# ZAX130/SmileCode

Measured on AMD Instinct MI355X. Metric: volume-pairs/sec (160x192x160) fwd+bwd, higher is better.
Workload: dtype f32; 1 GPU; ModeT 160x192x160 fp32, batch=1/GPU, full train step NCC+Grad3d fwd+bwd+Adam-amsgrad; global_batch=1, parallelism=dp1, allreduce=one flat all-reduce after backward

## Files before the change

### smilecode_amd/_lib.py

```python
from __future__ import annotations

import ctypes as C
import os
import re

_HERE = os.path.dirname(os.path.abspath(__file__))
LIB_PATH = os.environ.get("MODET_HIP_LIB") or os.path.join(_HERE, "lib", "libmodet_hip.so")
HEADER_PATH = os.path.join(os.path.dirname(_HERE), "include", "modet_hip.h")

P, I, I64, F, SZ = C.c_void_p, C.c_int, C.c_int64, C.c_float, C.c_size_t

class LeafJob(C.Structure):
    _fields_ = [("part", P), ("outer", I64), ("outer_stride", I64), ("rows", I64), ("row_stride", I64),
                ("col_group_stride", I64), ("ncols", I), ("col_group", I), ("dst", P * 4), ("n", I * 4)]


SIGNATURES = {
    "modet_hip_version": (I, []),
    "modet_hip_strerror": (C.c_char_p, [I]),
    "modet_qk_fwd": (I, [P, P, P, P, I, I, I, I, I, I, P]),
    "modet_qk_bwd_ws_bytes": (SZ, [I, I, I, I, I]),
    "modet_qk_bwd": (I, [P, P, P, P, P, P, P, SZ, I, I, I, I, I, I, P]),
    "modet_qk_fwd_f64": (I, [P, P, P, P, I, I, I, I, I, I, P]),
    "modet_qk_bwd_ws_bytes_f64": (SZ, [I, I, I, I, I]),
# ... 114 lines not shown
def _header(name):
    return os.path.join(os.path.dirname(_HERE), "include", name)


FAMILIES = {
    "core": (HEADER_PATH, SIGNATURES),
    "mind": (_header("modet_hip_losses.h"), {
        "modet_mind_ws_bytes": (SZ, [I, I, I, I, I]),
        "modet_mind_descriptor": (I, [P, P, P, SZ, I, I, I, I, I, I, P]),
        "modet_mind_fwd_bwd": (I, [P, P, P, P, P, SZ, I, I, I, I, I, I, F, P]),
    }),
    "mi": (_header("modet_hip_mi.h"), {
        "modet_mi_ws_bytes": (SZ, [I, I, I, I, I]),
        "modet_mi_fwd_bwd": (I, [P, P, P, P, P, P, SZ, I, I, I, I, I, F, F, F, F, P]),
        "modet_lmi_fwd_bwd": (I, [P, P, P, P, P, P, SZ, I, I, I, I, I, F, F, F, I, F, P]),
    }),
    "ssim": (_header("modet_hip_ssim.h"), {
        "modet_ssim_ws_bytes": (SZ, [I, I, I, I, I]),
        "modet_ssim_fwd_bwd": (I, [P, P, P, P, P, P, SZ, I, I, I, I, I, F, P]),
    }),
    "reg": (_header("modet_hip_reg.h"), {
        "modet_reg_ws_bytes": (SZ, [I, I, I, I, I, I]),
        "modet_reg_fwd_bwd": (I, [P, P, P, P, SZ, I, I, I, I, I, I, I, F, P]),
    }),
    "vecint": (_header("modet_hip_vecint.h"), {
        "modet_vecint_fwd": (I, [P, P, P, P, I, I, I, I, I, P]),
        "modet_vecint_ws_bytes": (SZ, [I, I, I, I, I, F]),
        "modet_vecint_bwd": (I, [P, P, P, P, P, P, SZ, I, I, I, I, I, F, P]),
    }),
    "surface": (_header("modet_hip_surface.h"), {
        "modet_surface_ws_bytes": (SZ, [I, I, I, I]),
        "modet_surface_distances": (I, [P, P, P, P, P, SZ, I, I, I, I, F, P]),
    }),
}
((LOSS_HEADER_PATH, LOSS_SIGNATURES), (MI_HEADER_PATH, MI_SIGNATURES), (SSIM_HEADER_PATH, SSIM_SIGNATURES),
 (REG_HEADER_PATH, REG_SIGNATURES), (VECINT_HEADER_PATH, VECINT_SIGNATURES)) = (FAMILIES[k] for k in ("mind", "mi", "ssim", "reg", "vecint"))

_lib = None


def header_symbols(path=None):
    txt = open(path or HEADER_PATH).read()
    txt = re.sub(r"/\*.*?\*/", "", txt, flags=re.S)
    return sorted(set(re.findall(r"\b(modet_[a-z0-9_]+)\s*\(", txt)))


def load():
    global _lib
    if _lib is not None:
        return _lib
    if not os.path.exists(LIB_PATH):
        raise RuntimeError(
            f"{LIB_PATH} not found: build it with `python -m smilecode_amd.build` "
            "(the ModeT hot path has no CPU / eager fallback)")
    lib = C.CDLL(LIB_PATH)
    for _, table in FAMILIES.values():
        for name, (res, args) in table.items():
            if not hasattr(lib, name) and os.environ.get("MODET_HIP_LIB"):
                continue
            fn = getattr(lib, name)
            fn.restype = res
            fn.argtypes = args
    _lib = lib
    return lib


# ... 8 lines not shown
```

### smilecode_amd/csrc/na.hip

```cpp
#include "common.h"
#include "drpb_reduce.h"
#include <cstdlib>

namespace {

constexpr int HD = 6;
constexpr int TZ = 4, TY = 4, TX = 16;
constexpr int HZ = TZ + 2, HY = TY + 2, HX = TX + 2;
constexpr int HVOX = HZ * HY * HX;
constexpr int NTHREADS = TZ * TY * TX;

struct TileGeom {
  int tiles_x, tiles_y, tiles_z;
};

__device__ __forceinline__ void tile_origin(int tile, const TileGeom g, int& z0, int& y0, int& x0) {
  const int tx = tile % g.tiles_x;
  const int t2 = tile / g.tiles_x;
  x0 = tx * TX;
  y0 = (t2 % g.tiles_y) * TY;
  z0 = (t2 / g.tiles_y) * TZ;
}

constexpr int KT_IT = (HVOX * 3 + NTHREADS - 1) / NTHREADS;
__device__ __forceinline__ float2 bf2_unpack(unsigned u) { return make_float2(__uint_as_float(u << 16), __uint_as_float(u & 0xffff0000u)); }
template <bool QK16 = false>
__device__ __forceinline__ void stage_k_load(float2 (&r)[KT_IT], const float* __restrict__ k, int64_t bbase, int z0, int y0,
                                             int x0, int D, int H, int W, int C, int hoff) {
  bool inside[KT_IT];
#pragma unroll
  for (int j = 0; j < KT_IT; ++j) {
    const int idx = min((int)threadIdx.x + j * NTHREADS, HVOX * 3 - 1);
    const int v = idx / 3, part = idx - v * 3;
    const int hx = v % HX, t = v / HX;
// ... 45 lines not shown
}

__device__ __forceinline__ void logits27(const float* __restrict__ kt, int lt, const float (&qs)[HD],
                                         const float* __restrict__ rpb_h, float (&lg)[27]) {
#pragma unroll
  for (int ki = 0; ki < 3; ++ki)
#pragma unroll
    for (int kj = 0; kj < 3; ++kj)
#pragma unroll
      for (int kk = 0; kk < 3; ++kk) {
        const int t = ki * 9 + kj * 3 + kk;
        float kv[HD];
        load6(kt + (lt + (ki * HY + kj) * HX + kk) * HD, kv);
        float s = rpb_h[t];
#pragma unroll
        for (int c = 0; c < HD; ++c) s = fmaf(qs[c], kv[c], s);
        lg[t] = s;
      }
}

__device__ __forceinline__ float softmax27(float (&lg)[27], float& m) {
  m = lg[0];
#pragma unroll
  for (int t = 1; t < 27; ++t) m = fmaxf(m, lg[t]);
  float s = 0.f;
#pragma unroll
  for (int t = 0; t < 27; ++t) {
    lg[t] = __expf(lg[t] - m);
    s += lg[t];
  }
  return 1.f / s;
}

template <bool QK16>
__global__ __launch_bounds__(NTHREADS) void na_fwd_kernel(const float* __restrict__ q, const float* __restrict__ k,
                                                          const float* __restrict__ rpb, float* __restrict__ out,
                                                          float* __restrict__ lse, int D, int H, int W, int heads,
                                                          float scale, TileGeom g) {
  __shared__ __attribute__((aligned(16))) float kt[HVOX * HD];
  __shared__ float rp[27];
  const int h = blockIdx.y, b = blockIdx.z;
  const int C = heads * HD;
  const int64_t V = (int64_t)D * H * W;
  int z0, y0, x0;
  tile_origin(blockIdx.x, g, z0, y0, x0);
  if (threadIdx.x < 27) rp[threadIdx.x] = rpb[h * 27 + threadIdx.x];
  stage_k_tile<QK16>(kt, k, (int64_t)b * V, z0, y0, x0, D, H, W, C, h * HD);
  __syncthreads();

  const int tx = threadIdx.x % TX, ty = (threadIdx.x / TX) % TY, tz = threadIdx.x / (TX * TY);
  const int z = z0 + tz, y = y0 + ty, x = x0 + tx;
  if (z >= D || y >= H || x >= W) return;
  const int64_t n = (int64_t)b * V + ((int64_t)z * H + y) * W + x;
  float qs[HD];
  load6g<QK16>(q, n * C + h * HD, qs);
#pragma unroll
  for (int c = 0; c < HD; ++c) qs[c] *= scale;
  float p[27];
  logits27(kt, (tz * HY + ty) * HX + tx, qs, rp, p);
  float mx;
  const float inv = softmax27(p, mx);
  if (lse) lse[n * heads + h] = mx - __logf(inv);
  float o0 = 0.f, o1 = 0.f, o2 = 0.f;
#pragma unroll
  for (int ki = 0; ki < 3; ++ki)
#pragma unroll
    for (int kj = 0; kj < 3; ++kj)
#pragma unroll
      for (int kk = 0; kk < 3; ++kk) {
        const float pv = p[ki * 9 + kj * 3 + kk];
        o0 += pv * (float)(ki - 1);
        o1 += pv * (float)(kj - 1);
        o2 += pv * (float)(kk - 1);
      }
  float* o = out + n * (heads * 3) + h * 3;
  o[0] = o0 * inv; o[1] = o1 * inv; o[2] = o2 * inv;
}

template <int N>
__device__ __forceinline__ void rs_step(float (&v)[32], int lane) {
  const bool up = (lane & N) != 0;
#pragma unroll
  for (int i = 0; i < N / 2; ++i) {
    const float keep = up ? v[i + N / 2] : v[i];
    const float send = up ? v[i] : v[i + N / 2];
    v[i] = keep + __shfl_xor(send, N, 64);
  }
}
__device__ __forceinline__ float wave_reduce_scatter32(const float (&v27)[27], int lane) {
  float v[32];
#pragma unroll
  for (int i = 0; i < 32; ++i) v[i] = i < 27 ? v27[i] : 0.f;
  rs_step<32>(v, lane); rs_step<16>(v, lane); rs_step<8>(v, lane); rs_step<4>(v, lane); rs_step<2>(v, lane);
  return v[0] + __shfl_xor(v[0], 1, 64);
}

constexpr int AUX = 5;

template <bool QK16>
__global__ __launch_bounds__(NTHREADS) void na_bwd_kernel(const float* __restrict__ q, const float* __restrict__ k,
                                                          const float* __restrict__ rpb, const float* __restrict__ out,
                                                          const float* __restrict__ lse, const float* __restrict__ dout,
                                                          float* __restrict__ dq, float* __restrict__ dk,
                                                          float* __restrict__ drpb_part, int D, int H, int W, int heads,
                                                          float scale, TileGeom g) {
  __shared__ __attribute__((aligned(16))) float kt[HVOX * HD];
  __shared__ __attribute__((aligned(16))) float qt[HVOX * HD];
  __shared__ float ax[HVOX * AUX];
  __shared__ float red[27 * (NTHREADS / 64)];
// ... 336 lines not shown
  const int lane = threadIdx.x & 63, wv = threadIdx.x >> 6;
  {
    const float r = wave_reduce_scatter32(dlv, lane);
    if ((lane & 1) == 0 && (lane >> 1) < 27) red[wv * 27 + (lane >> 1)] = r;
  }
  __syncthreads();
  if (threadIdx.x < 27) {
    float s = 0.f;
    for (int w = 0; w < NTHREADS / 64; ++w) s += red[w * 27 + threadIdx.x];
    const int64_t blk = ((int64_t)b * gridDim.y + h) * gridDim.x + blockIdx.x;
    a.drpb_part[blk * 27 + threadIdx.x] = s;
  }
}

struct NaMarchPlan { int tiles_x, tiles_y, nchunk, zc; bool on; };
inline NaMarchPlan na_march_plan(int B, int D, int H, int W, int heads, int hd) {
  NaMarchPlan p;
  p.tiles_x = cdiv(W, MX); p.tiles_y = cdiv(H, MY);
  p.on = hd == HD && (int64_t)D * H * W >= 1500000 && (int64_t)H * W * heads * HD * 4 < 0x7fffffffLL;
  const int cols = B * heads * p.tiles_x * p.tiles_y;
  int want = 2000;
#ifdef MODET_TUNING
  if (const char* e = getenv("MODET_NA_WGS")) want = atoi(e);
  if (const char* e = getenv("MODET_NA_MARCH")) p.on = p.on && e[0] != '0';
#endif
  int best = (want + cols - 1) / cols;
  const int maxn = D / 8 > 0 ? D / 8 : 1;
  best = best < 1 ? 1 : (best > maxn ? maxn : best);
  p.zc = cdiv(D, best);
  p.nchunk = cdiv(D, p.zc);
  return p;
}

constexpr int GC = 8;

__device__ __forceinline__ void stage_chunk(float* __restrict__ dst, const float* __restrict__ srcp, int64_t bbase, int z0,
                                            int y0, int x0, int D, int H, int W, int C, int coff) {
  for (int idx = threadIdx.x; idx < HVOX * 2; idx += NTHREADS) {
    const int v = idx >> 1, part = idx & 1;
    const int hx = v % HX, t = v / HX;
    const int hy = t % HY, hz = t / HY;
    const int z = z0 + hz - 1, y = y0 + hy - 1, x = x0 + hx - 1;
    float4 val = make_float4(0.f, 0.f, 0.f, 0.f);
    if (z >= 0 && z < D && y >= 0 && y < H && x >= 0 && x < W)
      val = *reinterpret_cast<const float4*>(srcp + (bbase + ((int64_t)z * H + y) * W + x) * C + coff + part * 4);
    *reinterpret_cast<float4*>(dst + v * GC + part * 4) = val;
  }
}
__device__ __forceinline__ void load8(const float* __restrict__ p, float (&r)[GC]) {
  const float4 a = *reinterpret_cast<const float4*>(p), b = *reinterpret_cast<const float4*>(p + 4);
  r[0] = a.x; r[1] = a.y; r[2] = a.z; r[3] = a.w; r[4] = b.x; r[5] = b.y; r[6] = b.z; r[7] = b.w;
}
__device__ __forceinline__ float dot8(const float (&a)[GC], const float (&b)[GC]) {
  float s = 0.f;
#pragma unroll
  for (int c = 0; c < GC; ++c) s = fmaf(a[c], b[c], s);
  return s;
}

__global__ __launch_bounds__(NTHREADS) void na_fwd_gen_kernel(const float* __restrict__ q, const float* __restrict__ k,
                                                              const float* __restrict__ rpb, float* __restrict__ out,
                                                              float* __restrict__ lse, int D, int H, int W, int heads,
                                                              int hd, float scale, TileGeom g) {
  __shared__ __attribute__((aligned(16))) float kt[HVOX * GC];
  __shared__ float rp[27];
  const int h = blockIdx.y, b = blockIdx.z;
// ... 164 lines not shown
            for (int c = 0; c < GC; ++c) dka[c] = fmaf(dlk[t], v8[c], dka[c]);
          }
      float* dqp = dq + n * C + h * hd + c0;
      float* dkp = dk + n * C + h * hd + c0;
      *reinterpret_cast<float4*>(dqp) = make_float4(dqa[0] * scale, dqa[1] * scale, dqa[2] * scale, dqa[3] * scale);
      *reinterpret_cast<float4*>(dqp + 4) = make_float4(dqa[4] * scale, dqa[5] * scale, dqa[6] * scale, dqa[7] * scale);
      *reinterpret_cast<float4*>(dkp) = make_float4(dka[0] * scale, dka[1] * scale, dka[2] * scale, dka[3] * scale);
      *reinterpret_cast<float4*>(dkp + 4) = make_float4(dka[4] * scale, dka[5] * scale, dka[6] * scale, dka[7] * scale);
    }
  }
  __syncthreads();
  if (threadIdx.x < 27) {
    float t = 0.f;
    for (int w = 0; w < NTHREADS / 64; ++w) t += red[w * 27 + threadIdx.x];
    const int64_t blk = ((int64_t)b * gridDim.y + h) * gridDim.x + blockIdx.x;
    drpb_part[blk * 27 + threadIdx.x] = t;
  }
}

inline bool gen_hd_ok(int hd) { return hd >= GC && hd <= 128 && hd % GC == 0; }

inline TileGeom geom(int D, int H, int W) { return TileGeom{cdiv(W, TX), cdiv(H, TY), cdiv(D, TZ)}; }

}

extern "C" {

int modet_na_fwd_t(const void* q, const void* k, int qk_bf16, const float* rpb, float* out, float* lse, int B, int D, int H, int W,
                   int heads, int hd, float scale, modet_stream_t stream) {
  if (!qk_bf16) return modet_na_fwd((const float*)q, (const float*)k, rpb, out, lse, B, D, H, W, heads, hd, scale, stream);
  MODET_CHECK_PTR(q); MODET_CHECK_PTR(k); MODET_CHECK_PTR(rpb); MODET_CHECK_PTR(out);
  MODET_CHECK_DIM(B > 0 && D > 0 && H > 0 && W > 0 && heads > 0);
  if (hd != HD) return MODET_ERR_UNSUPPORTED;
  const TileGeom g = geom(D, H, W);
  dim3 grid(g.tiles_x * g.tiles_y * g.tiles_z, heads, B);
  hipLaunchKernelGGL(na_fwd_kernel<true>, grid, dim3(NTHREADS), 0, (hipStream_t)stream, (const float*)q, (const float*)k, rpb, out,
                     lse, D, H, W, heads, scale, g);
  return modet_launch_status();
}

int modet_na_fwd(const float* q, const float* k, const float* rpb, float* out, float* lse, int B, int D, int H, int W,
                 int heads, int hd, float scale, modet_stream_t stream) {
  MODET_CHECK_PTR(q); MODET_CHECK_PTR(k); MODET_CHECK_PTR(rpb); MODET_CHECK_PTR(out);
  MODET_CHECK_DIM(B > 0 && D > 0 && H > 0 && W > 0 && heads > 0);
  if (hd != HD && !gen_hd_ok(hd)) return MODET_ERR_UNSUPPORTED;
  const TileGeom g = geom(D, H, W);
  dim3 grid(g.tiles_x * g.tiles_y * g.tiles_z, heads, B);
  if (hd == HD)
    hipLaunchKernelGGL(na_fwd_kernel<false>, grid, dim3(NTHREADS), 0, (hipStream_t)stream, q, k, rpb, out, lse, D, H, W, heads,
                       scale, g);
  else
    hipLaunchKernelGGL(na_fwd_gen_kernel, grid, dim3(NTHREADS), 0, (hipStream_t)stream, q, k, rpb, out, lse, D, H, W,
                       heads, hd, scale, g);
  return modet_launch_status();
}

size_t modet_na_bwd_ws_bytes(int B, int D, int H, int W, int heads) {
  const TileGeom g = geom(D, H, W);
  size_t fl = (size_t)B * heads * g.tiles_x * g.tiles_y * g.tiles_z * 27;
  fl += fl & 1;
  return fl * sizeof(float) + drpb_scratch_bytes(B, heads);
}

int modet_na_bwd_t(const void* qv, const void* kv, int qk_bf16, const float* rpb, const float* out, const float* lse,
                   const float* d_out, float* d_q, float* d_k, float* d_rpb, void* ws, size_t ws_bytes, int B, int D,
                   int H, int W, int heads, int hd, float scale, modet_stream_t stream) {
  const float* q = (const float*)qv;
  const float* k = (const float*)kv;
  MODET_CHECK_PTR(q); MODET_CHECK_PTR(k); MODET_CHECK_PTR(rpb); MODET_CHECK_PTR(out); MODET_CHECK_PTR(lse);
  MODET_CHECK_PTR(d_out); MODET_CHECK_PTR(d_q); MODET_CHECK_PTR(d_k); MODET_CHECK_PTR(ws);
  MODET_CHECK_DIM(B > 0 && D > 0 && H > 0 && W > 0 && heads > 0);
  if (hd != HD && (qk_bf16 || !gen_hd_ok(hd))) return MODET_ERR_UNSUPPORTED;
  if (ws_bytes < modet_na_bwd_ws_bytes(B, D, H, W, heads)) return MODET_ERR_WORKSPACE;
  hipStream_t s = (hipStream_t)stream;
  const NaMarchPlan mp = na_march_plan(B, D, H, W, heads, hd);
  if (mp.on) {
    const int64_t nblk = (int64_t)mp.tiles_x * mp.tiles_y * mp.nchunk;
    NaMarchArgs a{q, k, rpb, out, lse, d_out, d_q, d_k, (float*)ws, D, H, W, heads, mp.tiles_x, mp.tiles_y, mp.nchunk, mp.zc, scale};
// ... 1 lines not shown
    else hipLaunchKernelGGL(na_bwd_march_kernel<false>, dim3((unsigned)nblk, heads, B), dim3(NTHREADS), 0, s, a);
    size_t fl = (size_t)B * heads * nblk * 27;
    fl += fl & 1;
    if (d_rpb) drpb_reduce((float*)ws, ws, fl * sizeof(float), d_rpb, B, heads, nblk, s);
    return modet_launch_status();
  }
  const TileGeom g = geom(D, H, W);
  const int64_t nblk = (int64_t)g.tiles_x * g.tiles_y * g.tiles_z;
  float* part = (float*)ws;
  dim3 grid((unsigned)nblk, heads, B);
  if (hd == HD) {
    if (qk_bf16) hipLaunchKernelGGL(na_bwd_kernel<true>, grid, dim3(NTHREADS), 0, s, q, k, rpb, out, lse, d_out, d_q, d_k, part, D, H, W,
                                    heads, scale, g);
    else hipLaunchKernelGGL(na_bwd_kernel<false>, grid, dim3(NTHREADS), 0, s, q, k, rpb, out, lse, d_out, d_q, d_k, part, D, H, W,
                            heads, scale, g);
  } else {
    hipLaunchKernelGGL(na_bwd_gen_kernel, grid, dim3(NTHREADS), 0, s, q, k, rpb, out, lse, d_out, d_q, d_k, part, D, H, W,
                       heads, hd, scale, g);
  }
  size_t fl = (size_t)B * heads * nblk * 27;
  fl += fl & 1;
  if (d_rpb) drpb_reduce(part, ws, fl * sizeof(float), d_rpb, B, heads, nblk, s);
  return modet_launch_status();
}

int64_t modet_na_bwd_partial_rows(int B, int D, int H, int W, int heads, int hd) {
  if (B <= 0 || D <= 0 || H <= 0 || W <= 0 || heads <= 0) return 0;
  const NaMarchPlan mp = na_march_plan(B, D, H, W, heads, hd);
  if (mp.on) return (int64_t)mp.tiles_x * mp.tiles_y * mp.nchunk;
  const TileGeom g = geom(D, H, W);
  return (int64_t)g.tiles_x * g.tiles_y * g.tiles_z;
}

int modet_na_bwd(const float* q, const float* k, const float* rpb, const float* out, const float* lse,
                 const float* d_out, float* d_q, float* d_k, float* d_rpb, void* ws, size_t ws_bytes, int B, int D,
                 int H, int W, int heads, int hd, float scale, modet_stream_t stream) {
  return modet_na_bwd_t(q, k, 0, rpb, out, lse, d_out, d_q, d_k, d_rpb, ws, ws_bytes, B, D, H, W, heads, hd, scale, stream);
}

}
```

### smilecode_amd/csrc/proj_ln.hip

```cpp
#include "common.h"

namespace {

constexpr int BLK = 256;
constexpr int MAXW = 48 * 128;

__device__ __forceinline__ float4 ld4x(const float* __restrict__ base, int64_t el, bool x16) {
  if (x16) {
    const uint2 u = *reinterpret_cast<const uint2*>(reinterpret_cast<const unsigned short*>(base) + el);
    return make_float4(__uint_as_float(u.x << 16), __uint_as_float(u.x & 0xffff0000u), __uint_as_float(u.y << 16),
                       __uint_as_float(u.y & 0xffff0000u));
  }
  return *reinterpret_cast<const float4*>(base + el);
}
__device__ __forceinline__ unsigned short bf16_rne(float v) {
  const __bf16 b = (__bf16)v;
  return __builtin_bit_cast(unsigned short, b);
}

template <int DIM, bool X16 = false>
__device__ __forceinline__ void linear_ln(const float* __restrict__ xbase, int64_t xel, const float* __restrict__ Ws ,
                                          const float* __restrict__ bs, int Cin, float eps, float (&zh)[DIM],
                                          float& rstd) {
  float z[DIM];
#pragma unroll
  for (int o = 0; o < DIM; ++o) z[o] = bs[o];
  for (int c = 0; c < Cin; c += 4) {
    const float4 xv = ld4x(xbase, xel + c, X16);
    const float xs[4] = {xv.x, xv.y, xv.z, xv.w};
#pragma unroll
    for (int j = 0; j < 4; ++j)
#pragma unroll
      for (int o = 0; o < DIM; ++o) z[o] = fmaf(xs[j], Ws[(c + j) * DIM + o], z[o]);
  }
  float mu = 0.f;
#pragma unroll
  for (int o = 0; o < DIM; ++o) mu += z[o];
  mu *= (1.f / DIM);
  float var = 0.f;
#pragma unroll
  for (int o = 0; o < DIM; ++o) { const float d = z[o] - mu; var = fmaf(d, d, var); }
  rstd = rsqrtf(var * (1.f / DIM) + eps);
#pragma unroll
  for (int o = 0; o < DIM; ++o) zh[o] = (z[o] - mu) * rstd;
}

__device__ __forceinline__ void stage_w(float* Ws, float* ps, const float* __restrict__ Wt,
                                        const float* __restrict__ p0, const float* __restrict__ p1,
                                        const float* __restrict__ p2, int Cin, int DIM) {
  for (int i = threadIdx.x; i < Cin * DIM; i += BLK) {
    const int o = i / Cin, c = i - o * Cin;
    Ws[c * DIM + o] = Wt[i];
  }
  for (int i = threadIdx.x; i < DIM; i += BLK) {
    ps[i] = p0[i];
    if (p1) ps[DIM + i] = p1[i];
    if (p2) ps[2 * DIM + i] = p2[i];
  }
}

template <int DIM, bool X16 = false, bool Y16 = false>
__global__ __launch_bounds__(BLK) void proj_ln_fwd_kernel(const float* __restrict__ x, const float* __restrict__ Wt,
                                                          const float* __restrict__ bias, const float* __restrict__ gamma,
                                                          const float* __restrict__ beta, float* __restrict__ y,
                                                          int64_t N, int Cin, float eps) {
  extern __shared__ __attribute__((aligned(16))) float smem[];
  float* Ws = smem;
  float* ps = smem + Cin * DIM;
  stage_w(Ws, ps, Wt, bias, gamma, beta, Cin, DIM);
  __syncthreads();
  for (int64_t n = (int64_t)blockIdx.x * BLK + threadIdx.x; n < N; n += (int64_t)gridDim.x * BLK) {
    float zh[DIM], rstd;
    linear_ln<DIM, X16>(x, n * Cin, Ws, ps, Cin, eps, zh, rstd);
    float* yp = y + n * DIM;
#pragma unroll
    for (int o = 0; o < DIM; o += 2) {
      float2 v;
      v.x = fmaf(zh[o], ps[DIM + o], ps[2 * DIM + o]);
      v.y = fmaf(zh[o + 1], ps[DIM + o + 1], ps[2 * DIM + o + 1]);
      if constexpr (Y16) reinterpret_cast<unsigned*>(y)[(n * DIM + o) >> 1] = (unsigned)bf16_rne(v.x) | ((unsigned)bf16_rne(v.y) << 16);
      else *reinterpret_cast<float2*>(yp + o) = v;
    }
  }
}

template <int DIM, int CIN_REG>
__global__ __launch_bounds__(BLK) void proj_ln_bwd_kernel(const float* __restrict__ x, const float* __restrict__ Wt,
                                                          const float* __restrict__ bias, const float* __restrict__ gamma,
                                                          const float* __restrict__ dy, float* __restrict__ dx,
                                                          float* __restrict__ dz_out, float* __restrict__ part,
                                                          int64_t N, int Cin, float eps) {
// ... 701 lines not shown
```

### smilecode_amd/models.py

```python
from __future__ import annotations

import math

import torch
import torch.nn as nn

from . import ops


class _SplitBatch(torch.autograd.Function):

    @staticmethod
    def forward(ctx, x, B):
        ctx.B = B
        return x[:B], x[B:]

    @staticmethod
    def backward(ctx, ga, gb):
        B = ctx.B
        ref = ga if ga is not None else gb
        out = torch.empty((2 * B,) + tuple(ref.shape[1:]), dtype=ref.dtype, device=ref.device)
        if ga is None:
            out[:B].zero_()
        else:
# ... 383 lines not shown
    def forward_cl(self, moving, fixed):
        if moving.shape != fixed.shape or moving.dim() != 5:
            raise RuntimeError("ModeT.forward expects two (B,C,D,H,W) volumes of the same shape")
        if any(int(v) % 16 != 0 for v in moving.shape[2:]):
            raise RuntimeError(f"ModeT.forward: every spatial dimension must be a multiple of 16 (four 2x poolings, then x2 "
                               f"upsampling back: the level sizes would not match), got {tuple(moving.shape[2:])}")
        B = moving.shape[0]
        mov_cl = ops.to_channels_last(moving.contiguous())
        fix_cl = ops.to_channels_last(fixed.contiguous())
        with ops.trace_range("encoder"):
            M, Fx = self.encoder.forward_pair(ops.cat_batch(mov_cl, fix_cl), B, handles=self.level_bf16)
        if self.stage_cuts:
            self.cut_features = (M, Fx)
            M = [ops.feature_handle_like(m.detach().requires_grad_(True), m) for m in M]
            Fx = [ops.feature_handle_like(f.detach().requires_grad_(True), f) for f in Fx]
            self.cut_leaves = (M, Fx)
        ST = self.transformer
        if self.diff:
            integ = lambda lvl, w, bound=0.0: self.integrate[lvl].forward_cl(w, bound)
        else:
            integ = lambda lvl, w, bound=0.0: w

        def match(lvl, proj, mdt, flow):
            if self.level_bf16 and mdt.fused and mdt.use_rpb:
                res = ops.level_attention_bf16(Fx[lvl], M[lvl], flow, proj.proj.weight, proj.proj.bias, proj.norm.weight,
                                               proj.norm.bias, mdt.rpb, mdt.num_heads, mdt.scale, tee=flow is not None)
                return res if flow is not None else (res, None)
            if getattr(Fx[lvl], "data16", None) is not None:
                raise RuntimeError("ModeT: bf16 level features are only readable by the fused level nodes")
            if flow is None:
                Mw = M[lvl]
            else:
                Mw, flow = ops.warp_tee(M[lvl], flow)
            q, k = proj.forward_pair(Fx[lvl], Mw)
            return mdt(q, k), flow

        with ops.trace_range("level5"):
            flow = integ(4, self.cwm5(match(4, self.projblock5, self.mdt5, None)[0]))

        with ops.trace_range("level4"):
            field, flow = match(3, self.projblock4, self.mdt4, flow)
            w = integ(3, self.cwm4(field))
            flow = ST[2].forward_cl(ops.upsample2(flow, 2.0), w, add_flow=True)

        with ops.trace_range("level3"):
            field, flow = match(2, self.projblock3, self.mdt3, flow)
            w = integ(2, self.cwm3(field))
            flow = ST[1].forward_cl(ops.upsample2(flow, 2.0), w, add_flow=True)

        with ops.trace_range("level2"):
            w, flow = match(1, self.projblock2, self.mdt2, flow)
            w = integ(1, w, 1.0)
            flow = ops.upsample2(ST[1].forward_cl(flow, w, add_flow=True, flow_bound=1), 2.0)

        with ops.trace_range("level1"):
            w, flow = match(0, self.projblock1, self.mdt1, flow)
            w = integ(0, w, 1.0)
            flow = ST[0].forward_cl(flow, w, add_flow=True, flow_bound=1)
            y_moved, flow = ops.warp_tee(mov_cl, flow)
        return y_moved, flow


class ModeT_cu(ModeT):

    _flavour = "v"

# ... 12 lines not shown
```

### smilecode_amd/ops.py

```python
from __future__ import annotations

import ctypes
import os
import threading

import torch
from torch.autograd import Function

from . import _lib

LRELU_SLOPE = 0.1


def _L():
    return _lib.load()


def _stream():
    return torch.cuda.current_stream().cuda_stream


def _call(fn, *args):
    _lib.check(fn(*args), fn.__name__)

# ... 1005 lines not shown
    if heads < 1 or C % heads != 0:
        raise RuntimeError(f"{op}: {C} channels do not split into {heads} heads")
    hd = C // heads
    if hd != 6 and (bf16 or hd % 8 != 0 or hd > 128):
        raise RuntimeError(f"{op}: head_dim {hd} is not supported (6" + ("" if bf16 else ", or a multiple of 8 up to 128") + ")")
    if rpb.numel() != heads * 27:
        raise RuntimeError(f"{op}: rpb {tuple(rpb.shape)} does not hold {heads} x 27 biases")
    return hd


class _NA(Function):
    @staticmethod
    def forward(ctx, q, k, rpb, heads, scale):
        _chk(q, k, rpb)
        if q.dim() != 5:
            raise RuntimeError(f"neighbourhood attention: expects channels-last (B,D,H,W,heads*head_dim) q and k, got {tuple(q.shape)}")
        if k.shape != q.shape:
            raise RuntimeError("neighbourhood attention: q and k shapes differ")
        _na_args("neighbourhood attention", q.shape[-1], heads, rpb, False)
        need_grad = any(ctx.needs_input_grad[:3])
        out, lse = _na_fwd(q, k, rpb, heads, scale, need_grad)
        if need_grad:
            ctx.save_for_backward(q, k, rpb, out, lse)
        ctx.heads, ctx.scale = heads, float(scale)
        ctx.step = current_step()
        return out

    @staticmethod
    def backward(ctx, dout):
        q, k, rpb, out, lse = ctx.saved_tensors
        (drpb,), later, ret = _param_dsts(ctx.step, rpb)
        dq, dk = _na_bwd(q, k, rpb, out, lse, dout.contiguous(), ctx.heads, ctx.scale, ctx.step, drpb, later)
        return dq, dk, ret[0], None, None


class _LevelAttnBF16(Function):

    @staticmethod
    def forward(ctx, F, M, flow, Wt, b, gamma, beta, rpb, heads, scale, eps, tee=False):
        _chk(Wt, b, gamma, beta, rpb)
        ctx.tee = bool(tee) and flow is not None
        ctx.set_materialize_grads(False)
        ctx.step = current_step()
        ctx.beta_ref = beta
        _rank5("level attention (bf16)", "F", F)
        B, D, H, W, Cin = F.shape
        dim = Wt.shape[0]
        _same_shape("level attention (bf16)", "M", M, F.shape, "F")
        _same_shape("level attention (bf16)", "flow", flow, (B, D, H, W, 3), f"F {tuple(F.shape)}")
        _proj_args("level attention (bf16)", Cin, Wt, b, gamma, beta)
        _na_args("level attention (bf16)", dim, heads, rpb, True)
        N = B * D * H * W
        L = _L()
        n = float(N)
        Fd, Md = getattr(F, "data16", None), getattr(M, "data16", None)
        Fd = F if Fd is None else Fd
        Md = M if Md is None else Md
        _chk16(Fd, Md)
        _same_shape("level attention (bf16)", "F's bf16 data", Fd, F.shape, "F")
        _same_shape("level attention (bf16)", "M's bf16 data", Md, M.shape, "M")
        m16 = int(Md.dtype == torch.bfloat16)
        if flow is not None:
            _chk(flow)
            Mw = torch.empty(M.shape, dtype=torch.bfloat16, device=M.device)
            with _Guard(M, f"warp_fwd[C{Cin}]", n * (24.0 * Cin + 30.0), n * ((2.0 if m16 else 4.0) * Cin + 2.0 * Cin + 12.0)):
                _call(L.modet_warp_fwd_t, _p(Md), m16, _p(flow), _p(Mw), 1, B, D, H, W, Cin, _stream())
# ... 1072 lines not shown
```

Before: 141.6 volume-pairs/sec.

## Fuse projection+LayerNorm into z-marching neighbourhood attention forward kernel

Adds a z-marching forward kernel for neighbourhood attention that keeps three k-planes in a shared-memory ring buffer. It also adds a fused variant that computes the q/k linear projection and LayerNorm from the raw features on the fly, writing q and k once for the backward pass. The model's level matching routes fp32 single-head levels through this fused path, and the existing NA forward entry points use the marching kernel on large volumes. This is meant to remove the separate proj_ln pass and the q/k re-reads, and to cut halo re-staging across z tiles. In exchange, the k projection is recomputed on halo voxels, there is more register pressure, and some cost sits in serial z-loop synchronisation.

```diff
diff --git a/include/modet_hip_attn.h b/include/modet_hip_attn.h
--- /dev/null
+++ b/include/modet_hip_attn.h
@@ -0,0 +1,18 @@
+#ifndef MODET_HIP_ATTN_H
+#define MODET_HIP_ATTN_H
+
+#include "modet_hip.h"
+
+#ifdef __cplusplus
+extern "C" {
+#endif
+
+int modet_level_attn_fwd_ok(int B, int D, int H, int W, int Cin, int heads, int head_dim);
+int modet_level_attn_fwd(const float* F, const float* Mw, const float* Wt, const float* bias, const float* gamma,
+                         const float* beta, const float* rpb, float* q, float* k, float* out, float* lse, int B, int D, int H,
+                         int W, int Cin, int heads, int head_dim, float scale, float eps, modet_stream_t stream);
+
+#ifdef __cplusplus
+}
+#endif
+#endif
diff --git a/smilecode_amd/_lib.py b/smilecode_amd/_lib.py
--- a/smilecode_amd/_lib.py
+++ b/smilecode_amd/_lib.py
@@ -170,6 +170,10 @@
         "modet_surface_ws_bytes": (SZ, [I, I, I, I]),
         "modet_surface_distances": (I, [P, P, P, P, P, SZ, I, I, I, I, F, P]),
     }),
+    "attn": (_header("modet_hip_attn.h"), {
+        "modet_level_attn_fwd_ok": (I, [I, I, I, I, I, I, I]),
+        "modet_level_attn_fwd": (I, [P, P, P, P, P, P, P, P, P, P, P, I, I, I, I, I, I, I, F, F, P]),
+    }),
 }
 ((LOSS_HEADER_PATH, LOSS_SIGNATURES), (MI_HEADER_PATH, MI_SIGNATURES), (SSIM_HEADER_PATH, SSIM_SIGNATURES),
  (REG_HEADER_PATH, REG_SIGNATURES), (VECINT_HEADER_PATH, VECINT_SIGNATURES)) = (FAMILIES[k] for k in ("mind", "mi", "ssim", "reg", "vecint"))
diff --git a/smilecode_amd/csrc/na.hip b/smilecode_amd/csrc/na.hip
--- a/smilecode_amd/csrc/na.hip
+++ b/smilecode_amd/csrc/na.hip
@@ -1,5 +1,7 @@
 #include "common.h"
 #include "drpb_reduce.h"
+#include "../../include/modet_hip_attn.h"
+#include "proj_ln_device.h"
 #include <cstdlib>
 
 namespace {
@@ -111,11 +113,48 @@
   return 1.f / s;
 }
 
-template <bool QK16>
+__device__ __forceinline__ void na_fwd_finish(float (&p)[27], int64_t n, int heads, int h, float* __restrict__ out,
+                                              float* __restrict__ lse) {
+  float mx;
+  const float inv = softmax27(p, mx);
+  if (lse) lse[n * heads + h] = mx - __logf(inv);
+  float o0 = 0.f, o1 = 0.f, o2 = 0.f;
+#pragma unroll
+  for (int ki = 0; ki < 3; ++ki)
+#pragma unroll
+    for (int kj = 0; kj < 3; ++kj)
+#pragma unroll
+      for (int kk = 0; kk < 3; ++kk) {
+        const float pv = p[ki * 9 + kj * 3 + kk];
+        o0 += pv * (float)(ki - 1);
+        o1 += pv * (float)(kj - 1);
+        o2 += pv * (float)(kk - 1);
+      }
+  float* o = out + n * (heads * 3) + h * 3;
+  o[0] = o0 * inv; o[1] = o1 * inv; o[2] = o2 * inv;
+}
+
+struct NaFwdMarchArgs {
+  const float* q; const float* k;
+  const float* Wt; const float* bias; const float* gamma; const float* beta;
+  float* qo; float* ko;
+  const float* rpb; float* out; float* lse;
+  int D, H, W, heads, tiles_x, tiles_y, ZC;
+  float scale, eps;
+};
+template <int CIN, bool QK16>
+__device__ __forceinline__ void na_fwd_march(const NaFwdMarchArgs& a);
+
+template <bool QK16, bool MARCH = false>
 __global__ __launch_bounds__(NTHREADS) void na_fwd_kernel(const float* __restrict__ q, const float* __restrict__ k,
                                                           const float* __restrict__ rpb, float* __restrict__ out,
                                                           float* __restrict__ lse, int D, int H, int W, int heads,
                                                           float scale, TileGeom g) {
+  if constexpr (MARCH) {
+    na_fwd_march<0, QK16>(NaFwdMarchArgs{q, k, nullptr, nullptr, nullptr, nullptr, nullptr, nullptr, rpb, out, lse, D, H, W, heads,
+                                         g.tiles_x, g.tiles_y, g.tiles_z, scale, 0.f});
+    return;
+  }
   __shared__ __attribute__((aligned(16))) float kt[HVOX * HD];
   __shared__ float rp[27];
   const int h = blockIdx.y, b = blockIdx.z;
@@ -137,23 +176,7 @@
   for (int c = 0; c < HD; ++c) qs[c] *= scale;
   float p[27];
   logits27(kt, (tz * HY + ty) * HX + tx, qs, rp, p);
-  float mx;
-  const float inv = softmax27(p, mx);
-  if (lse) lse[n * heads + h] = mx - __logf(inv);
-  float o0 = 0.f, o1 = 0.f, o2 = 0.f;
-#pragma unroll
-  for (int ki = 0; ki < 3; ++ki)
-#pragma unroll
-    for (int kj = 0; kj < 3; ++kj)
-#pragma unroll
-      for (int kk = 0; kk < 3; ++kk) {
-        const float pv = p[ki * 9 + kj * 3 + kk];
-        o0 += pv * (float)(ki - 1);
-        o1 += pv * (float)(kj - 1);
-        o2 += pv * (float)(kk - 1);
-      }
-  float* o = out + n * (heads * 3) + h * 3;
-  o[0] = o0 * inv; o[1] = o1 * inv; o[2] = o2 * inv;
+  na_fwd_finish(p, n, heads, h, out, lse);
 }
 
 template <int N>
@@ -556,6 +579,208 @@
   return p;
 }
 
+constexpr int MFSLOT = MHV * HD;
+static_assert(BLK == NTHREADS, "stage_w strides by BLK");
+
+__device__ __forceinline__ void logits27_planes(const float* __restrict__ k0, const float* __restrict__ k1,
+                                                const float* __restrict__ k2, int hc, const float (&qs)[HD],
+                                                const float (&rp)[27], float (&lg)[27]) {
+#pragma unroll
+  for (int ki = 0; ki < 3; ++ki) {
+    const float* kt = ki == 0 ? k0 : (ki == 1 ? k1 : k2);
+#pragma unroll
+    for (int kj = 0; kj < 3; ++kj)
+#pragma unroll
+      for (int kk = 0; kk < 3; ++kk) {
+        const int t = ki * 9 + kj * 3 + kk;
+        float kv[HD];
+        load6(kt + (hc + (kj - 1) * MHX + (kk - 1)) * HD, kv);
+        float s = rp[t];
+#pragma unroll
+        for (int c = 0; c < HD; ++c) s = fmaf(qs[c], kv[c], s);
+        lg[t] = s;
+      }
+  }
+}
+
+template <int CIN, bool QK16>
+__device__ __forceinline__ void na_fwd_march(const NaFwdMarchArgs& a) {
+  constexpr bool FUSED = CIN > 0;
+  static_assert(!(FUSED && QK16) && CIN % 4 == 0, "the fused front end reads fp32 features");
+  __shared__ __attribute__((aligned(16))) float ring[3 * MFSLOT + (FUSED ? CIN * HD + 3 * HD : 0)];
+  float* Ws = ring + 3 * MFSLOT;
+  float* ps = Ws + CIN * HD;
+  const int h = blockIdx.y, b = blockIdx.z;
+  const int D = a.D, H = a.H, W = a.W, heads = a.heads;
+  const int C = heads * HD;
+  int t = blockIdx.x;
+  const int x0 = (t % a.tiles_x) * MX; t /= a.tiles_x;
+  const int y0 = (t % a.tiles_y) * MY;
+  const int zs = (t / a.tiles_y) * a.ZC;
+  const int ze = zs + a.ZC < D ? zs + a.ZC : D;
+  float rp[27];
+#pragma unroll
+  for (int i = 0; i < 27; ++i) rp[i] = a.rpb[h * 27 + i];
+  if constexpr (FUSED) stage_w(Ws, ps, a.Wt, a.bias, a.gamma, a.beta, CIN, HD);
+
+  const int64_t V = (int64_t)D * H * W, HW = (int64_t)H * W;
+  constexpr int QSZ = QK16 ? 2 : 4;
+  const int row = FUSED ? CIN * 4 : C * QSZ;
+  const int64_t first = FUSED ? (int64_t)b * V * CIN * 4 : ((int64_t)b * V * C + h * HD) * QSZ;
+  const char* qb = reinterpret_cast<const char*>(a.q) + first;
+  const char* kb = reinterpret_cast<const char*>(a.k) + first;
+  const unsigned pbytes = (unsigned)(HW * row);
+
+  constexpr int NIT = (MHV + NTHREADS - 1) / NTHREADS;
+  constexpr int NX = FUSED ? CIN : HD;
+  unsigned ok_[NIT];
+  int sl_[NIT], own_[NIT];
+#pragma unroll
+  for (int j = 0; j < NIT; ++j) {
+    const int v = threadIdx.x + j * NTHREADS;
+    const bool on = v < MHV;
+    const int hy = on ? v / MHX : 0, hx = on ? v - hy * MHX : 0;
+    const int y = y0 + hy - 1, x = x0 + hx - 1;
+    const bool ok = on && y >= 0 && y < H && x >= 0 && x < W;
+    ok_[j] = ok ? (unsigned)(y * W + x) * (unsigned)row : NA_OOB;
+    sl_[j] = on ? v : -1;
+    own_[j] = (ok && hy >= 1 && hy <= MY && hx >= 1 && hx <= MX) ? y * W + x : -1;
+  }
+  const int tx = threadIdx.x % MX, ty = threadIdx.x / MX;
+  const int y = y0 + ty, x = x0 + tx;
+  const bool live = y < H && x < W;
+  const int hc = (ty + 1) * MHX + tx + 1;
+  const unsigned oown = live ? (unsigned)(y * W + x) * (unsigned)row : NA_OOB;
+
+  __attribute__((aligned(16))) float xk[NIT][NX];
+  __attribute__((aligned(16))) float xq[NX];
+  auto ld_row = [&](const NaBuf r, unsigned off, float* dst) {
+    if constexpr (FUSED) {
+#pragma unroll
+      for (int c = 0; c < CIN; c += 4) {
+        const float4 v4 = __builtin_bit_cast(float4, __builtin_amdgcn_raw_buffer_load_b128(r, (int)(off + c * 4), 0, 0));
+        dst[c] = v4.x; dst[c + 1] = v4.y; dst[c + 2] = v4.z; dst[c + 3] = v4.w;
+      }
+    } else {
+#pragma unroll
+      for (int c = 0; c < 3; ++c) {
+        float2 v2;
+        if constexpr (QK16) v2 = bf2_unpack(__builtin_amdgcn_raw_buffer_load_b32(r, (int)(off + c * 4), 0, 0));
+        else v2 = __builtin_bit_cast(float2, __builtin_amdgcn_raw_buffer_load_b64(r, (int)(off + c * 8), 0, 0));
+        dst[2 * c] = v2.x; dst[2 * c + 1] = v2.y;
+      }
+    }
+  };
+  auto load_plane = [&](int z) {
+    const bool pl = z >= 0 && z < D && z <= ze;
+    const int64_t zo = pl ? z : 0;
+    const NaBuf bk = na_rsrc(reinterpret_cast<const float*>(kb + zo * HW * row), pl ? pbytes : 0u);
+    const bool ql = z - 1 >= zs && z - 1 < ze;
+    const NaBuf bq = na_rsrc(reinterpret_cast<const float*>(qb + (ql ? z - 1 : 0) * HW * row), ql ? pbytes : 0u);
+#pragma unroll
+    for (int j = 0; j < NIT; ++j) ld_row(bk, ok_[j], xk[j]);
+    ld_row(bq, oown, xq);
+  };
+  float qs[HD];
+#pragma unroll
+  for (int o = 0; o < HD; ++o) qs[o] = 0.f;
+  auto store_plane = [&](int slot, int z) {
+    float* kt = ring + slot * MFSLOT;
+    const bool pl = z >= 0 && z < D && z <= ze, mine = z >= zs && z < ze;
+    const bool qmine = z - 1 >= zs && z - 1 < ze;
+#pragma unroll
+    for (int j = 0; j < NIT; ++j) {
+      if (sl_[j] < 0) continue;
+      float kr[HD];
+      if constexpr (FUSED) {
+#pragma unroll
+        for (int o = 0; o < HD; ++o) kr[o] = 0.f;
+        if (pl && ok_[j] != NA_OOB) {
+          float zh[HD], rstd;
+          linear_ln<HD>(xk[j], 0, Ws, ps, CIN, a.eps, zh, rstd);
+#pragma unroll
+          for (int o = 0; o < HD; ++o) kr[o] = fmaf(zh[o], ps[HD + o], ps[2 * HD + o]);
+          if (a.ko != nullptr && mine && own_[j] >= 0) {
+            float* kp = a.ko + ((int64_t)b * V + (int64_t)z * HW + own_[j]) * HD;
+#pragma unroll
+            for (int o = 0; o < HD; o += 2) *reinterpret_cast<float2*>(kp + o) = make_float2(kr[o], kr[o + 1]);
+          }
+        }
+      } else {
+#pragma unroll
+        for (int o = 0; o < HD; ++o) kr[o] = xk[j][o];
+      }
+#pragma unroll
+      for (int o = 0; o < HD; o += 2) *reinterpret_cast<float2*>(kt + sl_[j] * HD + o) = make_float2(kr[o], kr[o + 1]);
+    }
+    if (live && qmine) {
+      float qr[HD];
+      if constexpr (FUSED) {
+        float zh[HD], rstd;
+        linear_ln<HD>(xq, 0, Ws, ps, CIN, a.eps, zh, rstd);
+#pragma unroll
+        for (int o = 0; o < HD; ++o) qr[o] = fmaf(zh[o], ps[HD + o], ps[2 * HD + o]);
+        if (a.qo != nullptr) {
+          float* qp = a.qo + ((int64_t)b * V + (int64_t)(z - 1) * HW + (int64_t)y * W + x) * HD;
+#pragma unroll
+          for (int o = 0; o < HD; o += 2) *reinterpret_cast<float2*>(qp + o) = make_float2(qr[o], qr[o + 1]);
+        }
+      } else {
+#pragma unroll
+        for (int o = 0; o < HD; ++o) qr[o] = xq[o];
+      }
+#pragma unroll
+      for (int o = 0; o < HD; ++o) qs[o] = qr[o] * a.scale;
+    }
+  };
+
+  load_plane(zs - 1);
+  if constexpr (FUSED) __syncthreads();
+  store_plane(0, zs - 1);
+  load_plane(zs); store_plane(1, zs);
+  load_plane(zs + 1); store_plane(2, zs + 1);
+  load_plane(zs + 2);
+  __syncthreads();
+  for (int z = zs, i = 0; z < ze; ++z, ++i) {
+    const int s0 = i % 3, s1 = (i + 1) % 3, s2 = (i + 2) % 3;
+    if (live) {
+      float p[27];
+      logits27_planes(ring + s0 * MFSLOT, ring + s1 * MFSLOT, ring + s2 * MFSLOT, hc, qs, rp, p);
+      na_fwd_finish(p, (int64_t)b * V + ((int64_t)z * H + y) * W + x, heads, h, a.out, a.lse);
+    }
+    __syncthreads();
+    store_plane(s0, z + 2);
+    __syncthreads();
+    load_plane(z + 3);
+  }
+}
+
+template <int CIN>
+__global__ __launch_bounds__(NTHREADS, 2) void level_attn_fwd_kernel(const NaFwdMarchArgs a) {
+  na_fwd_march<CIN, false>(a);
+}
+
+inline NaMarchPlan level_attn_plan(int B, int D, int H, int W) {
+  NaMarchPlan p = na_march_plan(B, D, H, W, 1, HD);
+  const int cols = B * p.tiles_x * p.tiles_y;
+  int want = 2000, minz = 4;
+#ifdef MODET_TUNING
+  if (const char* e = getenv("MODET_LA_WGS")) want = atoi(e);
+  if (const char* e = getenv("MODET_LA_MINZ")) minz = atoi(e);
+#endif
+  int best = (want + cols - 1) / cols;
+  const int maxn = D / minz > 0 ? D / minz : 1;
+  best = best < 1 ? 1 : (best > maxn ? maxn : best);
+  p.zc = cdiv(D, best);
+  p.nchunk = cdiv(D, p.zc);
+  return p;
+}
+
+inline bool level_attn_ok(int B, int D, int H, int W, int Cin, int heads, int hd) {
+  return B > 0 && B <= 65535 && D > 0 && H > 0 && W > 0 && heads == 1 && hd == HD && (Cin == 8 || Cin == 16) &&
+         (int64_t)H * W * Cin * 4 < 0x7fffffffLL;
+}
+
 constexpr int GC = 8;
 
 __device__ __forceinline__ void stage_chunk(float* __restrict__ dst, const float* __restrict__ srcp, int64_t bbase, int z0,
@@ -786,6 +1011,13 @@
   MODET_CHECK_PTR(q); MODET_CHECK_PTR(k); MODET_CHECK_PTR(rpb); MODET_CHECK_PTR(out);
   MODET_CHECK_DIM(B > 0 && D > 0 && H > 0 && W > 0 && heads > 0);
   if (hd != HD) return MODET_ERR_UNSUPPORTED;
+  const NaMarchPlan mp = na_march_plan(B, D, H, W, heads, hd);
+  if (mp.on) {
+    hipLaunchKernelGGL((na_fwd_kernel<true, true>), dim3(mp.tiles_x * mp.tiles_y * mp.nchunk, heads, B), dim3(NTHREADS), 0,
+                       (hipStream_t)stream, (const float*)q, (const float*)k, rpb, out, lse, D, H, W, heads, scale,
+                       TileGeom{mp.tiles_x, mp.tiles_y, mp.zc});
+    return modet_launch_status();
+  }
   const TileGeom g = geom(D, H, W);
   dim3 grid(g.tiles_x * g.tiles_y * g.tiles_z, heads, B);
   hipLaunchKernelGGL(na_fwd_kernel<true>, grid, dim3(NTHREADS), 0, (hipStream_t)stream, (const float*)q, (const float*)k, rpb, out,
@@ -798,6 +1030,12 @@
   MODET_CHECK_PTR(q); MODET_CHECK_PTR(k); MODET_CHECK_PTR(rpb); MODET_CHECK_PTR(out);
   MODET_CHECK_DIM(B > 0 && D > 0 && H > 0 && W > 0 && heads > 0);
   if (hd != HD && !gen_hd_ok(hd)) return MODET_ERR_UNSUPPORTED;
+  const NaMarchPlan mp = na_march_plan(B, D, H, W, heads, hd);
+  if (mp.on) {
+    hipLaunchKernelGGL((na_fwd_kernel<false, true>), dim3(mp.tiles_x * mp.tiles_y * mp.nchunk, heads, B), dim3(NTHREADS), 0,
+                       (hipStream_t)stream, q, k, rpb, out, lse, D, H, W, heads, scale, TileGeom{mp.tiles_x, mp.tiles_y, mp.zc});
+    return modet_launch_status();
+  }
   const TileGeom g = geom(D, H, W);
   dim3 grid(g.tiles_x * g.tiles_y * g.tiles_z, heads, B);
   if (hd == HD)
@@ -865,6 +1103,25 @@
   return (int64_t)g.tiles_x * g.tiles_y * g.tiles_z;
 }
 
+int modet_level_attn_fwd_ok(int B, int D, int H, int W, int Cin, int heads, int head_dim) {
+  return level_attn_ok(B, D, H, W, Cin, heads, head_dim) ? 1 : 0;
+}
+
+int modet_level_attn_fwd(const float* F, const float* Mw, const float* Wt, const float* bias, const float* gamma,
+                         const float* beta, const float* rpb, float* q, float* k, float* out, float* lse, int B, int D, int H,
+                         int W, int Cin, int heads, int head_dim, float scale, float eps, modet_stream_t stream) {
+  MODET_CHECK_PTR(F); MODET_CHECK_PTR(Mw); MODET_CHECK_PTR(Wt); MODET_CHECK_PTR(bias); MODET_CHECK_PTR(gamma);
+  MODET_CHECK_PTR(beta); MODET_CHECK_PTR(rpb); MODET_CHECK_PTR(out);
+  MODET_CHECK_DIM(B > 0 && D > 0 && H > 0 && W > 0 && heads > 0 && Cin > 0 && head_dim > 0);
+  if (!level_attn_ok(B, D, H, W, Cin, heads, head_dim)) return MODET_ERR_UNSUPPORTED;
+  const NaMarchPlan mp = level_attn_plan(B, D, H, W);
+  const NaFwdMarchArgs a{F, Mw, Wt, bias, gamma, beta, q, k, rpb, out, lse, D, H, W, heads, mp.tiles_x, mp.tiles_y, mp.zc, scale, eps};
+  const dim3 grid(mp.tiles_x * mp.tiles_y * mp.nchunk, heads, B);
+  if (Cin == 8) hipLaunchKernelGGL(level_attn_fwd_kernel<8>, grid, dim3(NTHREADS), 0, (hipStream_t)stream, a);
+  else hipLaunchKernelGGL(level_attn_fwd_kernel<16>, grid, dim3(NTHREADS), 0, (hipStream_t)stream, a);
+  return modet_launch_status();
+}
+
 int modet_na_bwd(const float* q, const float* k, const float* rpb, const float* out, const float* lse,
                  const float* d_out, float* d_q, float* d_k, float* d_rpb, void* ws, size_t ws_bytes, int B, int D,
                  int H, int W, int heads, int hd, float scale, modet_stream_t stream) {
diff --git a/smilecode_amd/csrc/proj_ln.hip b/smilecode_amd/csrc/proj_ln.hip
--- a/smilecode_amd/csrc/proj_ln.hip
+++ b/smilecode_amd/csrc/proj_ln.hip
@@ -1,62 +1,13 @@
 #include "common.h"
+#include "proj_ln_device.h"
 
 namespace {
 
-constexpr int BLK = 256;
 constexpr int MAXW = 48 * 128;
 
-__device__ __forceinline__ float4 ld4x(const float* __restrict__ base, int64_t el, bool x16) {
-  if (x16) {
-    const uint2 u = *reinterpret_cast<const uint2*>(reinterpret_cast<const unsigned short*>(base) + el);
-    return make_float4(__uint_as_float(u.x << 16), __uint_as_float(u.x & 0xffff0000u), __uint_as_float(u.y << 16),
-                       __uint_as_float(u.y & 0xffff0000u));
-  }
-  return *reinterpret_cast<const float4*>(base + el);
-}
 __device__ __forceinline__ unsigned short bf16_rne(float v) {
   const __bf16 b = (__bf16)v;
   return __builtin_bit_cast(unsigned short, b);
-}
-
-template <int DIM, bool X16 = false>
-__device__ __forceinline__ void linear_ln(const float* __restrict__ xbase, int64_t xel, const float* __restrict__ Ws ,
-                                          const float* __restrict__ bs, int Cin, float eps, float (&zh)[DIM],
-                                          float& rstd) {
-  float z[DIM];
-#pragma unroll
-  for (int o = 0; o < DIM; ++o) z[o] = bs[o];
-  for (int c = 0; c < Cin; c += 4) {
-    const float4 xv = ld4x(xbase, xel + c, X16);
-    const float xs[4] = {xv.x, xv.y, xv.z, xv.w};
-#pragma unroll
-    for (int j = 0; j < 4; ++j)
-#pragma unroll
-      for (int o = 0; o < DIM; ++o) z[o] = fmaf(xs[j], Ws[(c + j) * DIM + o], z[o]);
-  }
-  float mu = 0.f;
-#pragma unroll
-  for (int o = 0; o < DIM; ++o) mu += z[o];
-  mu *= (1.f / DIM);
-  float var = 0.f;
-#pragma unroll
-  for (int o = 0; o < DIM; ++o) { const float d = z[o] - mu; var = fmaf(d, d, var); }
-  rstd = rsqrtf(var * (1.f / DIM) + eps);
-#pragma unroll
-  for (int o = 0; o < DIM; ++o) zh[o] = (z[o] - mu) * rstd;
-}
-
-__device__ __forceinline__ void stage_w(float* Ws, float* ps, const float* __restrict__ Wt,
-                                        const float* __restrict__ p0, const float* __restrict__ p1,
-                                        const float* __restrict__ p2, int Cin, int DIM) {
-  for (int i = threadIdx.x; i < Cin * DIM; i += BLK) {
-    const int o = i / Cin, c = i - o * Cin;
-    Ws[c * DIM + o] = Wt[i];
-  }
-  for (int i = threadIdx.x; i < DIM; i += BLK) {
-    ps[i] = p0[i];
-    if (p1) ps[DIM + i] = p1[i];
-    if (p2) ps[2 * DIM + i] = p2[i];
-  }
 }
 
 template <int DIM, bool X16 = false, bool Y16 = false>
diff --git a/smilecode_amd/csrc/proj_ln_device.h b/smilecode_amd/csrc/proj_ln_device.h
--- /dev/null
+++ b/smilecode_amd/csrc/proj_ln_device.h
@@ -0,0 +1,58 @@
+#pragma once
+#include "common.h"
+
+namespace {
+
+constexpr int BLK = 256;
+
+__device__ __forceinline__ float4 ld4x(const float* __restrict__ base, int64_t el, bool x16) {
+  if (x16) {
+    const uint2 u = *reinterpret_cast<const uint2*>(reinterpret_cast<const unsigned short*>(base) + el);
+    return make_float4(__uint_as_float(u.x << 16), __uint_as_float(u.x & 0xffff0000u), __uint_as_float(u.y << 16),
+                       __uint_as_float(u.y & 0xffff0000u));
+  }
+  return *reinterpret_cast<const float4*>(base + el);
+}
+
+template <int DIM, bool X16 = false>
+__device__ __forceinline__ void linear_ln(const float* __restrict__ xbase, int64_t xel, const float* __restrict__ Ws ,
+                                          const float* __restrict__ bs, int Cin, float eps, float (&zh)[DIM],
+                                          float& rstd) {
+  float z[DIM];
+#pragma unroll
+  for (int o = 0; o < DIM; ++o) z[o] = bs[o];
+  for (int c = 0; c < Cin; c += 4) {
+    const float4 xv = ld4x(xbase, xel + c, X16);
+    const float xs[4] = {xv.x, xv.y, xv.z, xv.w};
+#pragma unroll
+    for (int j = 0; j < 4; ++j)
+#pragma unroll
+      for (int o = 0; o < DIM; ++o) z[o] = fmaf(xs[j], Ws[(c + j) * DIM + o], z[o]);
+  }
+  float mu = 0.f;
+#pragma unroll
+  for (int o = 0; o < DIM; ++o) mu += z[o];
+  mu *= (1.f / DIM);
+  float var = 0.f;
+#pragma unroll
+  for (int o = 0; o < DIM; ++o) { const float d = z[o] - mu; var = fmaf(d, d, var); }
+  rstd = rsqrtf(var * (1.f / DIM) + eps);
+#pragma unroll
+  for (int o = 0; o < DIM; ++o) zh[o] = (z[o] - mu) * rstd;
+}
+
+__device__ __forceinline__ void stage_w(float* Ws, float* ps, const float* __restrict__ Wt,
+                                        const float* __restrict__ p0, const float* __restrict__ p1,
+                                        const float* __restrict__ p2, int Cin, int DIM) {
+  for (int i = threadIdx.x; i < Cin * DIM; i += BLK) {
+    const int o = i / Cin, c = i - o * Cin;
+    Ws[c * DIM + o] = Wt[i];
+  }
+  for (int i = threadIdx.x; i < DIM; i += BLK) {
+    ps[i] = p0[i];
+    if (p1) ps[DIM + i] = p1[i];
+    if (p2) ps[2 * DIM + i] = p2[i];
+  }
+}
+
+}
diff --git a/smilecode_amd/models.py b/smilecode_amd/models.py
--- a/smilecode_amd/models.py
+++ b/smilecode_amd/models.py
@@ -439,6 +439,11 @@
                 Mw = M[lvl]
             else:
                 Mw, flow = ops.warp_tee(M[lvl], flow)
+            if (mdt.fused and Mw.dtype == torch.float32 and Mw.dim() == 5 and
+                    ops.level_attention_ok(*Mw.shape, mdt.num_heads, mdt.head_dim)):
+                rpb = mdt.rpb if mdt.use_rpb else torch.zeros(mdt.num_heads, 3, 3, 3, dtype=Mw.dtype, device=Mw.device)
+                return ops.level_attention(Fx[lvl], Mw, proj.proj.weight, proj.proj.bias, proj.norm.weight, proj.norm.bias,
+                                           rpb, mdt.num_heads, mdt.scale), flow
             q, k = proj.forward_pair(Fx[lvl], Mw)
             return mdt(q, k), flow
 
diff --git a/smilecode_amd/ops.py b/smilecode_amd/ops.py
--- a/smilecode_amd/ops.py
+++ b/smilecode_amd/ops.py
@@ -1061,6 +1061,82 @@
         (drpb,), later, ret = _param_dsts(ctx.step, rpb)
         dq, dk = _na_bwd(q, k, rpb, out, lse, dout.contiguous(), ctx.heads, ctx.scale, ctx.step, drpb, later)
         return dq, dk, ret[0], None, None
+
+
+LEVEL_ATTN_FUSED = True
+
+
+def level_attention_ok(B, D, H, W, Cin, heads, head_dim):
+    return bool(_L().modet_level_attn_fwd_ok(B, D, H, W, Cin, heads, head_dim))
+
+
+def _level_attn_args(F, Mw, Wt, b, gamma, beta, rpb, heads):
+    op = "level attention"
+    _chk(F, Mw, Wt, b, gamma, beta, rpb)
+    _rank5(op, "F", F)
+    B, D, H, W, Cin = F.shape
+    _same_shape(op, "Mw", Mw, F.shape, "F")
+    _proj_args(op, Cin, Wt, b, gamma, beta)
+    dim = Wt.shape[0]
+    if isinstance(heads, bool) or not isinstance(heads, int) or heads < 1 or dim % heads != 0:
+        raise RuntimeError(f"{op}: {dim} channels do not split into {heads!r} heads")
+    if rpb.numel() != heads * 27:
+        raise RuntimeError(f"{op}: rpb {tuple(rpb.shape)} does not hold {heads} x 27 biases")
+    if F.numel() == 0:
+        raise RuntimeError(f"{op}: F {tuple(F.shape)} must be non-empty")
+    if not level_attention_ok(B, D, H, W, Cin, heads, dim // heads):
+        raise RuntimeError(f"{op}: heads {heads}, head_dim {dim // heads}, Cin {Cin} at {B}x{D}x{H}x{W} is not supported "
+                           "(one head of head_dim 6 over 8 or 16 input channels)")
+    return B, D, H, W, Cin, dim
+
+
+def _level_attn_fwd(F, Mw, Wt, b, gamma, beta, rpb, heads, scale, eps, need_grad):
+    B, D, H, W, Cin, dim = _level_attn_args(F, Mw, Wt, b, gamma, beta, rpb, heads)
+    dev = F.device
+    out = torch.empty((B, D, H, W, heads * 3), dtype=torch.float32, device=dev)
+    q = k = lse = None
+    if need_grad:
+        q = torch.empty((B, D, H, W, dim), dtype=torch.float32, device=dev)
+        k = torch.empty_like(q)
+        lse = torch.empty((B, D, H, W, heads), dtype=torch.float32, device=dev)
+    N = B * D * H * W
+    nvh = float(N) * heads
+    with _Guard(F, f"level_attn_fwd_kernel[{Cin}->{dim},h{heads}]", 2 * N * (2.0 * Cin * dim + 8.0 * dim) + 620.0 * nvh,
+                8.0 * N * (Cin + dim) + 60.0 * nvh):
+        _call(_L().modet_level_attn_fwd, _p(F), _p(Mw), _p(Wt), _p(b), _p(gamma), _p(beta), _p(rpb), _p(q), _p(k), _p(out), _p(lse),
+              B, D, H, W, Cin, heads, dim // heads, float(scale), float(eps), _stream())
+    return q, k, out, lse
+
+
+class _LevelAttn(Function):
+
+    @staticmethod
+    def forward(ctx, F, Mw, Wt, b, gamma, beta, rpb, heads, scale, eps):
+        need_grad = any(ctx.needs_input_grad)
+        q, k, out, lse = _level_attn_fwd(F, Mw, Wt, b, gamma, beta, rpb, heads, scale, eps, need_grad)
+        if need_grad:
+            ctx.save_for_backward(F, Mw, Wt, b, gamma, beta, rpb, q, k, out, lse)
+        ctx.heads, ctx.scale, ctx.eps = heads, float(scale), eps
+        ctx.step = current_step()
+        return out
+
+    @staticmethod
+    def backward(ctx, dout):
+        F, Mw, Wt, b, gamma, beta, rpb, q, k, out, lse = ctx.saved_tensors
+        (drpb,), later_r, ret_r = _param_dsts(ctx.step, rpb)
+        dq, dk = _na_bwd(q, k, rpb, out, lse, dout.contiguous(), ctx.heads, ctx.scale, ctx.step, drpb, later_r)
+        dsts, later_p, ret_p = _param_dsts(ctx.step, Wt, b, gamma, beta)
+        dF, dMw = _proj_pair_bwd(F, dq, Mw, dk, Wt, b, gamma, ctx.eps, ctx.step, dsts, later_p)
+        return (dF, dMw, *ret_p, ret_r[0], None, None, None)
+
+
+def level_attention(F, Mw, Wt, b, gamma, beta, rpb, heads, scale, eps=1e-5):
+    rpb = rpb.contiguous()
+    if not LEVEL_ATTN_FUSED:
+        _level_attn_args(F, Mw, Wt, b, gamma, beta, rpb, heads)
+        q, k = proj_ln_pair(F, Mw, Wt, b, gamma, beta, eps)
+        return neighbourhood_attention(q, k, rpb, heads, scale)
+    return _LevelAttn.apply(F, Mw, Wt, b, gamma, beta, rpb, heads, scale, eps)
 
 
 class _LevelAttnBF16(Function):
```

Result: no change. 142.8 volume-pairs/sec, median of 6 (+0.9%).
